# kongzhecn/OMG

Measured on AMD Instinct MI355X. Metric: images/sec @ SDXL 1024^2 50-step, 2-concept mask fusion, higher is better.
Workload: dtype fp16 (storage and MFMA operands; fp32 accumulate; = the reference's own torch_dtype, inference_lora.py:153-159).  Measured tolerance per UNet forward at full size vs the fp32 oracle: rms 1.09e-3, max 4.9e-3 of O(1) outputs — the reference's own fp16 eager execution, emulated op by op in the oracle

## Files before the change

### omg_amd/csrc/conv_f32_wino.hip

```cpp
#include "common.h"

namespace {

constexpr int WSTAGE = 16 * 2 * 64 * 16;
constexpr int WRAW = 3 * 4096;
constexpr int WLDS = 4 * WSTAGE + 2 * WRAW;
constexpr unsigned WINO_OOB = 0xfff00000u;

struct WinoP {
  const char* X; const char* U; const char* bias; const char* residual; char* Y;
  int Hin, Win, Cin, Hout, Wout, Cout, upsample;
  int py, px, nb;
  unsigned u_bytes;
};

typedef __attribute__((address_space(3))) void* wino_lds_ptr_t;

__device__ __forceinline__ void wino_dma16(__amdgpu_buffer_rsrc_t rs, char* lds, unsigned voff, int soff) {
  __builtin_amdgcn_raw_ptr_buffer_load_lds(rs, (wino_lds_ptr_t)lds, 16, (int)voff, soff, 0, 0);
}

__global__ __launch_bounds__(256, 1) void conv_f32_wino_kernel(WinoP p) {
  extern __shared__ __attribute__((aligned(16))) char smem[];
  const int tid = threadIdx.x, lane = tid & 63;
  const int w = __builtin_amdgcn_readfirstlane(tid >> 6);
  const int hi = lane >> 5, l31 = lane & 31;
  int bid = blockIdx.x;
  {
    const int nwg = gridDim.x;
    const int q = nwg >> 3, r = nwg & 7, xcd = bid & 7, idx = bid >> 3;
    bid = (xcd < r ? xcd * (q + 1) : r * (q + 1) + (xcd - r) * q) + idx;
  }
  const int nb = bid % p.nb;
  int t = bid / p.nb;
  const int bx = t % p.px; t /= p.px;
  const int by = t % p.py;
  const int b = t / p.py;
  const int Y0 = by * 16, X0 = bx * 16;

  const long img_bytes = (long)p.Hin * p.Win * p.Cin * 4;
  const __amdgpu_buffer_rsrc_t rsX = __builtin_amdgcn_make_buffer_rsrc((void*)(p.X + (long)b * img_bytes), 0,
                                                                      (int)(unsigned)(img_bytes < (long)WINO_OOB ? img_bytes : (long)WINO_OOB), 0x00020000);
  const __amdgpu_buffer_rsrc_t rsU = __builtin_amdgcn_make_buffer_rsrc((void*)p.U, 0, (int)p.u_bytes, 0x00020000);

  unsigned voffR[3];
  {
    const int Hl = p.upsample ? p.Hin * 2 : p.Hin, Wl = p.upsample ? p.Win * 2 : p.Win;
#pragma unroll
    for (int i = 0; i < 3; ++i) {
      const int s = i * 256 + tid, pixel = s >> 1, quad = s & 1;
      const int pr = pixel / 18;
      int iy = Y0 - 1 + pr, ix = X0 - 1 + (pixel - pr * 18);
      const bool ok = (pixel < 324) & ((unsigned)iy < (unsigned)Hl) & ((unsigned)ix < (unsigned)Wl);
      if (p.upsample) { iy >>= 1; ix >>= 1; }
      voffR[i] = ok ? ((unsigned)(iy * p.Win + ix) * (unsigned)p.Cin + (unsigned)quad * 4u) * 4u : WINO_OOB;
    }
  }
  const int nk = p.Cin >> 3;
  const unsigned voffU = (unsigned)tid * 16u;
  const int ubase = nb * nk;

  auto dma_x = [&](int rbuf, int kt) {
    char* dst = smem + 4 * WSTAGE + rbuf * WRAW + w * 1024;
#pragma unroll
    for (int i = 0; i < 3; ++i) wino_dma16(rsX, dst + i * 4096, voffR[i], kt * 32);
  };
  auto dma_u = [&](int buf, int kt) {
    char* dst = smem + (2 + buf) * WSTAGE + w * 1024;
    const int soff = (ubase + kt) * WSTAGE;
#pragma unroll
    for (int i = 0; i < 8; ++i) wino_dma16(rsU, dst + i * 4096, voffU + i * 4096u, soff);
  };
  const int cq = w & 1, half = w >> 1;
  const int offR = ((2 * (lane >> 3) + half) * 18 + 2 * (lane & 7)) * 32 + cq * 16;
  auto transform = [&](int buf, int rbuf) {
    const char* src = smem + 4 * WSTAGE + rbuf * WRAW + offR;
    f32x4 ta[4], tb[4];
#pragma unroll
    for (int c = 0; c < 4; ++c) {
      const f32x4 d0 = *(const f32x4*)(src + c * 32), d1 = *(const f32x4*)(src + (18 + c) * 32), d2 = *(const f32x4*)(src + (36 + c) * 32);
      if (half == 0) { ta[c] = d0 - d2; tb[c] = d1 + d2; }
      else           { ta[c] = d1 - d0; tb[c] = d0 - d2; }
    }
    char* dst = smem + buf * WSTAGE + (half * 8 * 2 + cq) * 1024 + lane * 16;
#pragma unroll
    for (int q = 0; q < 2; ++q) {
      const f32x4* tr = q ? tb : ta;
      *(f32x4*)(dst + (q * 4 + 0) * 2048) = tr[0] - tr[2];
      *(f32x4*)(dst + (q * 4 + 1) * 2048) = tr[1] + tr[2];
      *(f32x4*)(dst + (q * 4 + 2) * 2048) = tr[2] - tr[1];
      *(f32x4*)(dst + (q * 4 + 3) * 2048) = tr[1] - tr[3];
    }
  };

  const int wm = w >> 1, wn = w & 1;
  f32x16 acc[16];
#pragma unroll
  for (int i = 0; i < 16; ++i)
#pragma unroll
    for (int r = 0; r < 16; ++r) acc[i][r] = 0.f;

  const int offV = hi * 1024 + (wm * 32 + l31) * 16, offU = hi * 1024 + (wn * 32 + l31) * 16;
  auto mfmas = [&](int buf, int pos) {
    const f32x4 vf = *(const f32x4*)(smem + buf * WSTAGE + pos * 2048 + offV);
    const f32x4 uf = *(const f32x4*)(smem + (2 + buf) * WSTAGE + pos * 2048 + offU);
#pragma unroll
    for (int e = 0; e < 4; ++e) acc[pos] = __builtin_amdgcn_mfma_f32_32x32x2f32(uf[e], vf[e], acc[pos], 0, 0, 0);
  };

  dma_x(0, 0);
  dma_u(0, 0);
  asm volatile("s_waitcnt vmcnt(0)" ::: "memory");
  __syncthreads();
  transform(0, 0);
  if (nk > 1) dma_x(1, 1);
  for (int kt = 0; kt < nk; ++kt) {
    const int buf = kt & 1;
    asm volatile("s_waitcnt vmcnt(0)" ::: "memory");
    __syncthreads();
    if (kt + 1 < nk) dma_u(buf ^ 1, kt + 1);
    if (kt + 2 < nk) dma_x(buf, kt + 2);
    __builtin_amdgcn_sched_barrier(0);
#pragma unroll
    for (int pos = 0; pos < 4; ++pos) mfmas(buf, pos);
    __builtin_amdgcn_sched_barrier(0);
    if (kt + 1 < nk) transform(buf ^ 1, buf ^ 1);
    __builtin_amdgcn_sched_barrier(0);
#pragma unroll
    for (int pos = 4; pos < 16; ++pos) mfmas(buf, pos);
  }

  const int tile = wm * 32 + l31;
  const int oy = Y0 + 2 * (tile >> 3), ox = X0 + 2 * (tile & 7);
  if (oy >= p.Hout || ox >= p.Wout) return;
  const long pix = ((long)b * p.Hout + oy) * p.Wout + ox;
#pragma unroll
  for (int g = 0; g < 4; ++g) {
    const int c = nb * 64 + wn * 32 + g * 8 + hi * 4;
    if (c >= p.Cout) continue;
    f32x4 y[2][2];
#pragma unroll
    for (int q = 0; q < 4; ++q) {
      const int r = g * 4 + q;
      float s0[4], s1[4];
#pragma unroll
      for (int j = 0; j < 4; ++j) {
        s0[j] = acc[j][r] + acc[4 + j][r] + acc[8 + j][r];
        s1[j] = acc[4 + j][r] - acc[8 + j][r] - acc[12 + j][r];
      }
      y[0][0][q] = s0[0] + s0[1] + s0[2]; y[0][1][q] = s0[1] - s0[2] - s0[3];
      y[1][0][q] = s1[0] + s1[1] + s1[2]; y[1][1][q] = s1[1] - s1[2] - s1[3];
    }
    f32x4 bv = {0.f, 0.f, 0.f, 0.f};
    if (p.bias) bv = *(const f32x4*)(p.bias + (long)c * 4);
#pragma unroll
    for (int a = 0; a < 2; ++a)
#pragma unroll
      for (int e = 0; e < 2; ++e) {
        const long o = ((pix + (long)a * p.Wout + e) * p.Cout + c) * 4;
        f32x4 v = y[a][e] + bv;
        if (p.residual) v += *(const f32x4*)(p.residual + o);
        *(f32x4*)(p.Y + o) = v;
      }
  }
}

}

extern "C" int64_t omg_conv2d_f32_wino_weight_floats(int Cout, int Cin) {
  return (int64_t)((Cout + 63) / 64) * (Cin / 8) * (WSTAGE / 4);
}

extern "C" int omg_conv2d_f32_wino(const omg_conv2d_f32_wino_args* a, void* stream) {
  OMG_REQUIRE(a != nullptr, "omg_conv2d_f32_wino: null args");
  OMG_REQUIRE(a->Cin > 0 && a->Cin % 8 == 0 && a->Cout > 0 && a->Cout % 4 == 0, "omg_conv2d_f32_wino: Cin % 8, Cout % 4");
  OMG_REQUIRE(a->X && a->U && a->Y, "omg_conv2d_f32_wino: null operand");
  const int Hl = a->upsample ? 2 * a->Hin : a->Hin, Wl = a->upsample ? 2 * a->Win : a->Win;
  OMG_REQUIRE(a->Hout == Hl && a->Wout == Wl, "omg_conv2d_f32_wino: 3x3, stride 1, 'same' padding only");
  OMG_REQUIRE(a->Hout % 2 == 0 && a->Wout % 2 == 0, "omg_conv2d_f32_wino: even output sizes only (2x2 tiles)");
  if (a->B == 0 || a->Hout == 0 || a->Wout == 0) return OMG_OK;
  WinoP p{};
  p.X = (const char*)a->X; p.U = (const char*)a->U; p.bias = (const char*)a->bias; p.residual = (const char*)a->residual; p.Y = (char*)a->Y;
  p.Hin = a->Hin; p.Win = a->Win; p.Cin = a->Cin; p.Hout = a->Hout; p.Wout = a->Wout; p.Cout = a->Cout; p.upsample = a->upsample;
  p.py = (a->Hout + 15) / 16; p.px = (a->Wout + 15) / 16; p.nb = (a->Cout + 63) / 64;
  const long img_bytes = (long)a->Hin * a->Win * a->Cin * 4, u_bytes = (long)omg_conv2d_f32_wino_weight_floats(a->Cout, a->Cin) * 4;
  const long blocks = (long)a->B * p.py * p.px * p.nb;
  OMG_REQUIRE(img_bytes < (long)WINO_OOB && u_bytes < 0x7fffffffL && blocks < 0x7fffffffL,
              "omg_conv2d_f32_wino: an image / the weight image beyond the 32-bit offsets of the kernel");
  p.u_bytes = (unsigned)u_bytes;
  static bool attr = false;
  if (!attr) { attr = true; (void)hipFuncSetAttribute((const void*)conv_f32_wino_kernel, hipFuncAttributeMaxDynamicSharedMemorySize, WLDS); }
  OMG_LAUNCH(conv_f32_wino_kernel, dim3((unsigned)blocks), dim3(256), WLDS, (hipStream_t)stream, p);
  return omg_check_launch("conv2d_f32_wino");
}
```

Measured before the change: 0.4149.

## Interleave Winograd input transform with MFMAs and double-buffer LDS fragment loads

The Winograd input transform used to run as one block between MFMA groups. It is now split into per-MFMA slices: LDS loads of raw rows, then the ta/tb combines, then the stores. Each slice is placed after one MFMA with scheduling barriers, so LDS and VALU work hides under matrix latency. The V/U fragment reads are software-pipelined one position ahead, and the weight DMA moves its per-chunk offset into the scalar offset. The transform now also runs on the last k-step, which is wasted work. The tight sched_barrier placement may stop the compiler from finding a better order.

```diff
diff --git a/omg_amd/csrc/conv_f32_wino.hip b/omg_amd/csrc/conv_f32_wino.hip
--- a/omg_amd/csrc/conv_f32_wino.hip
+++ b/omg_amd/csrc/conv_f32_wino.hip
@@ -69,7 +69,7 @@
     char* dst = smem + (2 + buf) * WSTAGE + w * 1024;
     const int soff = (ubase + kt) * WSTAGE;
 #pragma unroll
-    for (int i = 0; i < 8; ++i) wino_dma16(rsU, dst + i * 4096, voffU + i * 4096u, soff);
+    for (int i = 0; i < 8; ++i) wino_dma16(rsU, dst + i * 4096, voffU, soff + i * 4096);
   };
   const int cq = w & 1, half = w >> 1;
   const int offR = ((2 * (lane >> 3) + half) * 18 + 2 * (lane & 7)) * 32 + cq * 16;
@@ -101,13 +101,10 @@
     for (int r = 0; r < 16; ++r) acc[i][r] = 0.f;
 
   const int offV = hi * 1024 + (wm * 32 + l31) * 16, offU = hi * 1024 + (wn * 32 + l31) * 16;
-  auto mfmas = [&](int buf, int pos) {
-    const f32x4 vf = *(const f32x4*)(smem + buf * WSTAGE + pos * 2048 + offV);
-    const f32x4 uf = *(const f32x4*)(smem + (2 + buf) * WSTAGE + pos * 2048 + offU);
-#pragma unroll
-    for (int e = 0; e < 4; ++e) acc[pos] = __builtin_amdgcn_mfma_f32_32x32x2f32(uf[e], vf[e], acc[pos], 0, 0, 0);
-  };
-
+
+  const int offT = offR - half * (18 * 32);
+  const int offX = (half ? 2 : 0) * (18 * 32), offY = (half ? 1 : 2) * (18 * 32), offZ = (half ? 3 : 1) * (18 * 32);
+  const float sz = half ? -1.f : 1.f;
   dma_x(0, 0);
   dma_u(0, 0);
   asm volatile("s_waitcnt vmcnt(0)" ::: "memory");
@@ -121,13 +118,37 @@
     if (kt + 1 < nk) dma_u(buf ^ 1, kt + 1);
     if (kt + 2 < nk) dma_x(buf, kt + 2);
     __builtin_amdgcn_sched_barrier(0);
-#pragma unroll
-    for (int pos = 0; pos < 4; ++pos) mfmas(buf, pos);
-    __builtin_amdgcn_sched_barrier(0);
-    if (kt + 1 < nk) transform(buf ^ 1, buf ^ 1);
-    __builtin_amdgcn_sched_barrier(0);
-#pragma unroll
-    for (int pos = 4; pos < 16; ++pos) mfmas(buf, pos);
+    const char* vb = smem + buf * WSTAGE + offV;
+    const char* ub = smem + (2 + buf) * WSTAGE + offU;
+    const char* tsrc = smem + 4 * WSTAGE + (buf ^ 1) * WRAW + offT;
+    char* tdst = smem + (buf ^ 1) * WSTAGE + (half * 8 * 2 + cq) * 1024 + lane * 16;
+    f32x4 vf[2], uf[2], dx[4], dy[4], dz[4], ta[4], tb[4];
+    vf[0] = *(const f32x4*)vb;
+    uf[0] = *(const f32x4*)ub;
+#pragma unroll
+    for (int pos = 0; pos < 16; ++pos) {
+      if (pos + 1 < 16) {
+        vf[(pos + 1) & 1] = *(const f32x4*)(vb + (pos + 1) * 2048);
+        uf[(pos + 1) & 1] = *(const f32x4*)(ub + (pos + 1) * 2048);
+      }
+      __builtin_amdgcn_sched_barrier(0);
+#pragma unroll
+      for (int e = 0; e < 4; ++e) {
+        const int m = pos * 4 + e;
+        acc[pos] = __builtin_amdgcn_mfma_f32_32x32x2f32(uf[pos & 1][e], vf[pos & 1][e], acc[pos], 0, 0, 0);
+        __builtin_amdgcn_sched_barrier(0);
+        if (m < 4) {
+          dx[m] = *(const f32x4*)(tsrc + offX + m * 32); dy[m] = *(const f32x4*)(tsrc + offY + m * 32); dz[m] = *(const f32x4*)(tsrc + offZ + m * 32);
+        } else if (m < 8) {
+          ta[m - 4] = dx[m - 4] - dy[m - 4]; tb[m - 4] = dy[m - 4] + dz[m - 4] * sz;
+        } else if (m < 16) {
+          const int o = m - 8, j = o & 3;
+          const f32x4* tr = o >> 2 ? tb : ta;
+          *(f32x4*)(tdst + o * 2048) = j == 0 ? tr[0] - tr[2] : j == 1 ? tr[1] + tr[2] : j == 2 ? tr[2] - tr[1] : tr[1] - tr[3];
+        }
+        __builtin_amdgcn_sched_barrier(0);
+      }
+    }
   }
 
   const int tile = wm * 32 + l31;
```

Result: no change. 0.4155 (median of 6 runs) (+0.1%).
